# iwbn/flow-supervisor

Measured on AMD Instinct MI355X. Metric: image-pairs/s fwd+bwd, 12 GRU iters, 436x1024, higher is better.
Workload: dtype f32 (bf16x3 products); 1 GPU; RAFT full, 440x1024 (Sintel 436x1024 padded), 12 GRU iters, 4 pairs/GPU, train step = fwd + sequence loss + bwd + RCCL all-reduce + clip + AdamW; global_batch=4, parallelism=dp1, launch=hipGraph replay of the whole step

## Files before the change

### flow_supervisor_amd/_lib.py

```python
import ctypes
import functools
import os
from ctypes import POINTER, Structure, c_double, c_float, c_int, c_int64, c_void_p

import torch

_HERE = os.path.dirname(os.path.abspath(__file__))
LIB_PATH = os.environ.get("FSRAFT_LIB_PATH") or os.path.join(_HERE, "libfsraft.so")
_lib = None

c_float_p = c_void_p


class ConvDesc(Structure):
    _fields_ = [
        ("src", c_void_p * 3), ("srcC", c_int * 3), ("srcld", c_int * 3), ("nsrc", c_int),
        ("wpk", c_void_p), ("bias", c_void_p), ("wpk_split", c_void_p),
        ("B", c_int), ("H", c_int), ("W", c_int), ("KH", c_int), ("KW", c_int), ("N", c_int),
        ("dst", c_void_p * 3), ("dst_bs", c_int64 * 3), ("dst_ps", c_int64 * 3), ("dst_cs", c_int64 * 3),
        ("dst_n0", c_int * 3), ("dst_acc", c_int * 3), ("ndst", c_int),
        ("relu", c_int), ("alpha", c_float),
        ("epi", c_int),
        ("h", c_void_p), ("ldh", c_int), ("z", c_void_p), ("ldz", c_int),
        ("aux1", c_void_p), ("ld1", c_int), ("aux2", c_void_p), ("ld2", c_int), ("hid", c_int),
        ("pre", c_void_p), ("ldpre", c_int),
        ("rmask", c_void_p * 3), ("ldmask", c_int * 3), ("maskc", c_int * 3),
        ("wpk_frag", c_void_p), ("pad_h1", c_int), ("pad_w1", c_int),
        ("ws", c_void_p), ("ws_floats", c_int64),
    ]


class PackJob(Structure):
    _fields_ = [
        ("w", c_void_p * 3), ("rows", c_int * 3), ("npiece", c_int),
        ("wpk", c_void_p),
        ("cin_full", c_int), ("kh", c_int), ("kw", c_int),
        ("srcC", c_int * 3), ("srcOff", c_int * 3), ("nsrc", c_int),
        ("mode", c_int), ("flags", c_int),
        ("scale", c_float), ("accumulate", c_int),
    ]


_PP = POINTER(c_void_p)
_IP = POINTER(c_int)
_S = c_void_p

SIGNATURES = {
    "fsraft_corr_build": [c_void_p, c_void_p, _PP, c_int, c_int, c_int, c_int, c_int, _S],
    "fsraft_corr_unpool_bwd": [_PP, c_int, c_int, c_int, c_int, _S],
    "fsraft_corr_lookup_fwd": [_PP, c_int, c_void_p, c_int64, c_int64, c_int64, c_void_p, c_int, c_int, c_int, c_int, c_int, _S],
    "fsraft_corr_lookup_bwd": [_PP, c_int, c_void_p, c_int64, c_int64, c_int64, c_void_p, c_int, c_int, c_int, c_int, c_int, _S],
    "fsraft_altcorr_fwd": [c_void_p, c_void_p, c_void_p, c_void_p, c_int, c_int, c_int, c_int, c_int, c_int, c_int, c_int, _S],
    "fsraft_altcorr_bwd": [c_void_p, c_void_p, c_void_p, c_void_p, c_void_p, c_void_p, c_int, c_int, c_int, c_int, c_int, c_int, c_int, c_int, _S],
    "fsraft_upsample_fwd": [c_void_p, c_int64, c_int64, c_int64, c_void_p, c_void_p, c_int, c_int, c_int, _S],
    "fsraft_upsample_bwd": [c_void_p, c_int64, c_int64, c_int64, c_void_p, c_void_p, c_void_p, c_void_p, c_void_p, c_int, c_int, c_int, _S],
    "fsraft_upflow8_fwd": [c_void_p, c_void_p, c_int, c_int, c_int, c_int, _S],
    "fsraft_upflow8_bwd": [c_void_p, c_void_p, c_int, c_int, c_int, c_int, _S],
    "fsraft_conv_ktot": [_IP, c_int, c_int, c_int],
    "fsraft_conv_forward": [POINTER(ConvDesc), _S],
    "fsraft_conv_forward_stats": [POINTER(ConvDesc), c_void_p, c_void_p, c_int, POINTER(c_int), _S],
    "fsraft_conv_wgrad": [c_void_p, c_int, c_int, _PP, _IP, _IP, c_int, c_void_p, c_void_p, c_int, c_int, c_int, c_int, c_int, _S],
    "fsraft_conv_wgrad_multi": [_PP, c_int, c_int, c_int, _PP, _IP, _IP, c_int, c_void_p, c_void_p, c_int, c_int, c_int, c_int, c_int, _S],
    "fsraft_conv_small_fwd": [c_void_p, c_int, c_int, c_void_p, c_void_p, c_void_p, c_int64, c_int64, c_int64, c_int, c_int, c_int, c_int, c_int, c_int, _S],
    "fsraft_conv_small_wgrad": [_PP, _PP, c_int, c_int, c_int, c_int, c_void_p, c_void_p, c_int, c_int, c_int, c_int, c_int, c_int, _S],
    "fsraft_conv_small_dgrad": [c_void_p, c_int, c_void_p, c_void_p, c_int, c_void_p, c_int, c_int, c_int, c_int, c_int, c_int, c_int, c_int, _S],
    "fsraft_pack_conv_weights": [POINTER(PackJob), c_int, _S],
    "fsraft_pack_conv_weight": [c_void_p, c_void_p, c_int, c_int, c_int, c_int, _IP, c_int, c_int, c_int, _S],
    "fsraft_set_rec_mfma16": [c_int],
    "fsraft_set_build_kernel": [c_int],
    "fsraft_set_dvol_policy": [c_int],
    "fsraft_set_dvol_box": [c_int],
    "fsraft_set_ktile_exact": [c_int],
    "fsraft_set_lookup_policy": [c_int],
    "fsraft_set_upsample_kernel": [c_int],
    "fsraft_conv_workspace": [c_void_p, c_int64],
    "fsraft_set_arithmetic": [c_int],
    "fsraft_get_arithmetic": [],
    "fsraft_set_tuning": [c_int, c_int],
    "fsraft_adamw_flat": [c_void_p, c_void_p, c_void_p, c_void_p, c_int64, c_void_p, c_void_p, c_float, c_void_p, c_double, c_double, c_float,
                          c_float, c_void_p, c_void_p, _S],
    "fsraft_stream_capture_id": [_S, c_void_p],
    "fsraft_stem_slots": [],
    "fsraft_stem7x7s2_fwd": [c_void_p, c_void_p, c_void_p, c_void_p, c_int, c_int, c_int, c_int, _S],
    "fsraft_stem7x7s2_wgrad": [c_void_p, c_void_p, c_void_p, c_void_p, c_int, c_int, c_int, c_int, _S],
    "fsraft_set_lookup_qb": [c_int],
    "fsraft_set_build_split": [c_int],
    "fsraft_set_gemm_split": [c_int],
    "fsraft_gemm_tn_split": [c_void_p, c_int64, c_int64, c_void_p, c_int64, c_int64, c_void_p, c_int64, c_int64, c_int, c_int, c_int, c_int, c_float, c_int, _S],
    "fsraft_gemm_f32": [c_void_p, c_int64, c_int64, c_void_p, c_int64, c_int64, c_void_p, c_int64, c_int64, c_int, c_int, c_int, c_int, c_int, c_float, c_int, _S],
    "fsraft_nchw_to_nhwc": [c_void_p, c_void_p, c_int, c_int, c_int, c_int, c_int, c_int, _S],
    "fsraft_nhwc_to_nchw": [c_void_p, c_void_p, c_int, c_int, c_int, c_int, c_int, c_int, _S],
    "fsraft_im2col7": [c_void_p, c_int64, c_int64, c_int64, c_void_p, c_int, c_int, c_int, c_int, _S],
    "fsraft_col2im7": [c_void_p, c_int, c_void_p, c_int, c_int, c_int, c_int, _S],
    "fsraft_flow_to_nhwc": [c_void_p, c_int64, c_int64, c_int64, c_void_p, c_int, c_int, c_int, c_int, _S],
    "fsraft_nhwc_to_flow": [c_void_p, c_int, c_int, c_void_p, c_int, c_int, c_int, _S],
    "fsraft_relu_bwd": [c_void_p, c_int, c_void_p, c_int, c_int64, c_int, _S],
    "fsraft_gru_bwd1": [c_void_p, c_void_p, c_void_p, c_void_p, c_void_p, c_void_p, c_int, c_void_p, c_void_p, c_void_p, c_void_p, c_int64, c_int, _S],
    "fsraft_gru_bwd2": [c_void_p, c_void_p, c_void_p, c_void_p, c_int, c_void_p, c_void_p, c_int64, c_int, _S],
    "fsraft_col_sum": [c_void_p, c_int, c_int64, c_int, c_void_p, c_float, _S],
    "fsraft_softmax_rows": [c_void_p, c_int64, c_int, _S],
    "fsraft_softmax_rows_bwd": [c_void_p, c_void_p, c_int64, c_int, _S],
    "fsraft_softmax_rows_rec": [c_void_p, c_int64, c_int, _S],
    "fsraft_softmax_rows_bwd_rec": [c_void_p, c_void_p, c_int64, c_int, _S],
    "fsraft_softmax_rows_pos": [c_void_p, c_void_p, c_int64, c_int64, c_int, c_int, c_int, c_int, c_int, _S],
    "fsraft_softmax_rows_pos_bwd": [c_void_p, c_void_p, c_void_p, c_int64, c_int64, c_int, c_int, c_int, c_int, _S],
    "fsraft_gma_mix_fwd": [c_void_p, c_int, c_void_p, c_int, c_void_p, c_void_p, c_int, c_int64, c_int, _S],
    "fsraft_gma_mix_bwd": [c_void_p, c_int, c_void_p, c_int, c_void_p, c_void_p, c_int, c_void_p, c_int, c_void_p, c_int64, c_int, _S],
    "fsraft_inorm_relu_fwd": [c_void_p, c_void_p, c_void_p, c_int64, c_int, c_float, c_int, _S],
    "fsraft_inorm_relu_bwd": [c_void_p, c_void_p, c_void_p, c_void_p, c_int64, c_int, c_int, _S],
    "fsraft_affine_relu_fwd": [c_void_p, c_void_p, c_void_p, c_void_p, c_int64, c_int, c_int, c_int, _S],
    "fsraft_affine_relu_bwd": [c_void_p, c_void_p, c_void_p, c_void_p, c_void_p, c_void_p, c_void_p, c_int64, c_int, c_int, c_int, _S],
    "fsraft_sequence_loss": [_PP, _PP, POINTER(c_float), c_int, c_int, c_void_p, c_void_p, c_float, c_float, c_int, c_int, c_int, c_void_p, _S],
    "fsraft_corr_pool_pyramid": [_PP, c_int, c_int64, c_int, c_int, _S],
    "fsraft_corr_pool_pyramid_same": [_PP, c_int, c_int64, c_int, c_int, _S],
    "fsraft_corr_lookup_fwd_same": [_PP, c_int, c_void_p, c_int64, c_int64, c_int64, c_void_p, c_int, c_int, c_int, c_int, c_int, _S],
    "fsraft_corr_unpool_same_bwd": [_PP, c_int, c_int64, c_int, c_int, _S],
    "fsraft_corr_lookup_bwd_same": [_PP, c_int, c_void_p, c_int64, c_int64, c_int64, c_void_p, c_int, c_int, c_int, c_int, c_int, _S],
    "fsraft_corr_lookup_dcoords_same": [_PP, c_int, c_void_p, c_int64, c_int64, c_int64, c_void_p, c_int, c_void_p, c_int64, c_int64, c_int64,
                                        c_int, c_int, c_int, c_int, _S],
    "fsraft_set_norm_blocks": [c_int],
    "fsraft_get_tuning": [c_int],
    "fsraft_conv_last_route": [c_int],
    "fsraft_set_wgrad_wide": [c_int],
    "fsraft_conv_wgrad_last_tile": [],
    "fsraft_space_to_depth2": [c_void_p, c_void_p, c_int, c_int, c_int, c_int, c_int, _S],
    "fsraft_forward_interpolate": [c_void_p, c_void_p, c_int, c_int, _S],
    "fsraft_flow_metrics_scratch_bytes": [c_int, c_int, c_int],
    "fsraft_flow_metrics": [c_void_p, c_int64, c_int64, c_int64, c_void_p, c_int64, c_int64, c_int64, c_void_p, c_int64, c_int64,
                            c_int, c_int, c_int, c_void_p, c_void_p, c_void_p, c_int64, _S],
    "fsraft_inorm_relu_cl_fwd": [c_void_p, c_void_p, c_void_p, c_void_p, c_void_p, c_void_p, c_int, c_int, c_int, c_float, c_int, c_int, c_int, _S],
    "fsraft_inorm_relu_cl_bwd": [c_void_p, c_void_p, c_void_p, c_void_p, c_void_p, c_void_p, c_void_p, c_void_p, c_int, c_int, c_int,
                                 c_int, c_int, _S],
    "fsraft_affine_relu_cl_fwd": [c_void_p, c_void_p, c_void_p, c_void_p, c_void_p, c_int64, c_int, c_int, c_int, c_int, _S],
    "fsraft_affine_relu_cl_bwd": [c_void_p, c_void_p, c_void_p, c_void_p, c_void_p, c_void_p, c_void_p, c_void_p, c_void_p, c_int, c_int,
                                  c_int, c_int, c_int, _S],
    "fsraft_axpby": [c_void_p, c_void_p, c_float, c_float, c_int64, _S],
    "fsraft_sum_n": [_PP, c_int, c_void_p, c_int64, c_int, _S],
    "fsraft_bn_fold": [c_void_p, c_void_p, c_void_p, c_void_p, c_void_p, c_float, c_int, c_void_p, c_void_p, c_void_p, c_void_p, _S],
    "fsraft_bn_fold_bwd": [c_void_p, c_int, c_int, c_void_p, c_void_p, c_void_p, c_void_p, c_void_p, c_void_p, _S],
    "fsraft_vol_layout": [c_int, c_int, c_int, _IP],
    "fsraft_corr_build_tiled": [c_void_p, c_void_p, c_void_p, c_int, c_int, c_int, c_int, c_int, _S],
    "fsraft_corr_build_rec": [c_void_p, c_void_p, c_void_p, c_int, c_int, c_int, c_int, c_int, _S],
    "fsraft_corr_lookup_tiled_fwd": [c_void_p, c_int, c_void_p, c_int64, c_int64, c_int64, c_void_p, c_int, c_int, c_int, c_int, c_int, _S],
    "fsraft_corr_lookup_tiled_dcoords": [c_void_p, c_int, c_void_p, c_int64, c_int64, c_int64, c_void_p, c_void_p, c_int64, c_int64, c_int64,
                                         c_int, c_int, c_int, c_int, c_int, _S],
    "fsraft_corr_lookup_dcoords": [_PP, c_int, c_void_p, c_int64, c_int64, c_int64, c_void_p, c_int, c_void_p, c_int64, c_int64, c_int64,
                                   c_int, c_int, c_int, c_int, _S],
    "fsraft_corr_dvol_build": [_PP, _PP, POINTER(c_int64), c_int, c_void_p, c_int, c_int, c_int, c_int, c_int, c_int, c_int, c_int, c_int64,
                               c_int64, c_void_p, c_void_p, _S],
    "fsraft_set_alt_tile": [c_int],
    "fsraft_altcorr_fused_fwd": [c_void_p, _PP, c_int, c_void_p, c_int64, c_int64, c_int64, c_int, c_void_p, c_int, c_int, c_int, c_int, c_int, _S],
    "fsraft_altcorr_fused_dcoords": [c_void_p, _PP, c_int, c_void_p, c_int64, c_int64, c_int64, c_int, c_void_p, c_void_p, c_int64, c_int64,
                                     c_int64, c_int, c_int, c_int, c_int, c_int, _S],
    "fsraft_altcorr_mfma_fwd": [c_void_p, _PP, c_void_p, _PP, c_int, c_void_p, c_int64, c_int64, c_int64, c_int, c_void_p, c_int, c_int, c_int, c_int, c_int, _S],
    "fsraft_corr_f2cat": [c_void_p, c_void_p, c_int, c_int, c_int, c_int, c_int, _S],
    "fsraft_corr_dfmap2": [c_void_p, c_void_p, c_int, c_int, c_int, c_int, c_int, _S],
    "fsraft_corr_f2cat_rec": [c_void_p, c_void_p, c_int, c_int, c_int, c_int, c_int, _S],
    "fsraft_to_records": [c_void_p, c_int64, c_void_p, c_int64, c_int64, c_int, _S],
    "fsraft_gemm_rec_tn": [c_void_p, c_int64, c_int64, c_void_p, c_int64, c_int64, c_void_p, c_int64, c_int64, c_int, c_int, c_int, c_int,
                           c_float, c_int, c_int, _S],
    "fsraft_gemm_rec_nt": [c_void_p, c_int64, c_int64, c_void_p, c_int64, c_int64, c_void_p, c_int64, c_int64, c_int, c_int, c_int, c_int,
                           c_float, c_int, c_int, _S],
    "fsraft_gemm_rec_nt_list": [c_void_p, c_int64, c_int64, c_void_p, c_int64, c_int64, c_void_p, c_int64, c_int64, c_int, c_int, c_int, c_int,
                                c_float, c_int, c_int, c_void_p, c_void_p, c_int, c_int, _S],
    "fsraft_gemm_rec_tn_list": [c_void_p, c_int64, c_int64, c_void_p, c_int64, c_int64, c_void_p, c_int64, c_int64, c_int, c_int, c_int, c_int,
                                c_float, c_int, c_int, c_void_p, c_void_p, c_int, c_int, _S],
    "fsraft_corr_bwd_ktiles": [_PP, POINTER(c_int64), c_int, c_int, c_int, c_int, c_int, c_int, c_int, c_int64, c_int64, c_void_p, c_void_p,
                               c_int, c_void_p, c_void_p, c_void_p, c_int, c_void_p, _S],
}

CONV_ROUTES = {
    1: ("fwd.gemm32", "fp32"), 2: ("fwd.gemm64", "fp32"), 3: ("fwd.gemm64x128", "fp32"), 4: ("fwd.gemm128", "fp32"),
    5: ("fwd.gemm64x64", "fp32"), 6: ("fwd.gemm64x64k16", "fp32"), 7: ("fwd.gemm64x128k16", "fp32"),
    10: ("fwd.patch128x128", "bf16x3"), 11: ("fwd.patch256x128", "bf16x3"), 12: ("fwd.patch128x64", "bf16x3"),
    13: ("fwd.patch256x64", "bf16x3"), 20: ("fwd.halo21", "bf16x3"), 21: ("fwd.halo22", "bf16x3"),
    30: ("fwd.split64x256", "bf16x3"), 31: ("fwd.split256x64", "bf16x3"), 32: ("fwd.split256x128w16", "bf16x3"),
    33: ("fwd.split128x128w8", "bf16x3"), 34: ("fwd.split64x128", "bf16x3"), 35: ("fwd.split128x128", "bf16x3"),
}
CONV_ROUTES.update({c + 100: (n + "+ksplit", a) for c, (n, a) in list(CONV_ROUTES.items()) if c >= 30})
WGRAD_ROUTES = {
    1: ("wgrad.exact32", "fp32"), 2: ("wgrad.exact64x64", "fp32"), 3: ("wgrad.exact128", "fp32"),
    4: ("wgrad.split128", "bf16x3"), 5: ("wgrad.split128S", "bf16x3"), 6: ("wgrad.pack", "bf16x3"),
    7: ("wgrad.patch", "bf16x3"), 8: ("wgrad.multi", "bf16x3"), 9: ("wgrad.multi_w8", "bf16x3"),
}


def load():
    global _lib
    if _lib is not None:
        return _lib
    if not os.path.exists(LIB_PATH):
        raise RuntimeError(
            f"{LIB_PATH} not found: build it with `python -c 'import __graft_entry__ as g; g.build()'` "
            "(or `make -C flow_supervisor_amd/csrc`). There is no CPU/eager fallback for the RAFT hot path.")
    lib = ctypes.CDLL(LIB_PATH)
    for name, argtypes in SIGNATURES.items():
        fn = getattr(lib, name)
        fn.argtypes = argtypes
        fn.restype = c_int
    _lib = lib
    arith = os.environ.get("FSRAFT_ARITHMETIC")
    if arith is not None:
        lib.fsraft_set_arithmetic(int(arith))
    split = os.environ.get("FSRAFT_CONV_SPLIT")
    if split is not None:
        lib.fsraft_set_tuning(3, int(split))
    bsplit = os.environ.get("FSRAFT_BUILD_SPLIT")
    if bsplit is not None:
        lib.fsraft_set_build_split(int(bsplit))
    for kv in filter(None, os.environ.get("FSRAFT_TUNING", "").split(",")):
        key, val = (int(v) for v in kv.split("="))
        if lib.fsraft_set_tuning(key, val) != 0:
            raise RuntimeError(f"FSRAFT_TUNING: key {key} is not a tuning key of this libfsraft (include/fsraft_tuning.h)")
    wsplit = os.environ.get("FSRAFT_WGRAD_SPLIT")
    if wsplit is not None:
        lib.fsraft_set_tuning(4, int(wsplit))
    return lib


def stream():
    return c_void_p(torch.cuda.current_stream().cuda_stream)


def check(rc, what):
    if rc != 0:
        raise RuntimeError(f"libfsraft: {what} failed with status {rc} "
                           f"({'bad argument' if rc == 1 else 'kernel launch error'})")


def ptr(t):
    return c_void_p(t.data_ptr()) if t is not None else c_void_p(0)


def ptr_array(tensors):
    arr = (c_void_p * len(tensors))(*[t.data_ptr() for t in tensors])
    return ctypes.cast(arr, _PP), arr


def int_array(vals):
    return (c_int * len(vals))(*vals)


def require_cuda_f32(*tensors):
    dev = None
    for t in tensors:
        if t is None:
            continue
        if not t.is_cuda:
            raise RuntimeError("fsraft ops need CUDA (ROCm) tensors; the hot path has no CPU implementation")
        if t.dtype != torch.float32:
            raise RuntimeError(f"fsraft ops are fp32-only, got {t.dtype}")
        if dev is None:
            dev = t.device
        elif t.device != dev:
            raise RuntimeError(f"fsraft ops need all tensors on one device, got {dev} and {t.device}")
    if dev is not None and dev.index != torch.cuda.current_device():
        raise RuntimeError(f"fsraft op called with tensors on {dev} while cuda:{torch.cuda.current_device()} is the current device; "
                           f"wrap the call in `with torch.cuda.device({dev.index}):`")


def _first_cuda_device(values):
    for v in values:
        if isinstance(v, torch.Tensor):
            if v.is_cuda:
                return v.device
        elif isinstance(v, (list, tuple)):
            d = _first_cuda_device(v)
            if d is not None:
                return d
    return None


def on_tensor_device(fn):
    @functools.wraps(fn)
    def guarded(*args, **kwargs):
        dev = _first_cuda_device(args)
# ... 8 lines not shown
```

### flow_supervisor_amd/csrc/conv_igemm.hip

```cpp
#include "conv_common.hpp"

namespace {

__device__ __forceinline__ void tile_of_block(int swz, int& bx, int& by) {
  if (!swz) return;
  const int nx = gridDim.x, T = nx * gridDim.y, i = by * nx + bx;
  const int x = i & 7, q = T >> 3, r = T & 7;
  const int t = x * q + (x < r ? x : r) + (i >> 3);
  bx = t % nx; by = t / nx;
}

template <class Cfg>
struct ConvALoader {
  static constexpr int BM = Cfg::BM, BK = Cfg::BK, LD = Cfg::LDA;
  static constexpr int F4 = BK / 4;
  static constexpr int NF4 = BM * F4 / 256;
  static constexpr int NREG = NF4 * 4;
  static constexpr int NCH = NF4;
  const float* p0; const float* p1; const float* p2;
  int C0, C1, C2, ld0, ld1, ld2;
  int cpt0, cpt1, cpt2;
  int taps, KW, PH, PW, H, W;
  int py[NF4], px[NF4];
  int64_t pb[NF4];
// ... 812 lines not shown
      const int mkc = di == 0 ? a.maskc[0] : di == 1 ? a.maskc[1] : a.maskc[2];
      const int64_t b = m / HW, pix = m - b * HW;
      float* o = dp + b * dbs + pix * dps + (int64_t)(n - dn0) * dcs;
      for (int i = 0; i < nv; ++i) {
        float r = v[i] * a.alpha;
        if (a.relu) r = fmaxf(r, 0.f);
        if (dacc) r += o[i * dcs];
        if (mk && n - dn0 + i < mkc && mk[m * ldm + (n - dn0) + i] <= 0.f) r = 0.f;
        o[i * dcs] = r;
      }
    } else if (EPI == EPI_ZR) {
      const bool isz = n < a.hid;
      const int c = isz ? n : n - a.hid;
      if (a.pre) v += gload4(a.pre + m * a.ldpre + n);
#pragma unroll
      for (int i = 0; i < 4; ++i) v[i] = 1.0f / (1.0f + expf(-v[i]));
      if (isz) {
        *reinterpret_cast<f32x4*>(a.dst[0].p + m * a.dst[0].ps + c) = v;
      } else {
        const f32x4 hh = gload4(a.h + m * a.ldh + c);
        *reinterpret_cast<f32x4*>(a.aux2 + m * a.ld2 + c) = v;
        f32x4 rh;
#pragma unroll
        for (int i = 0; i < 4; ++i) rh[i] = v[i] * hh[i];
        *reinterpret_cast<f32x4*>(a.aux1 + m * a.ld1 + c) = rh;
      }
    } else {
      if (a.pre) v += gload4(a.pre + m * a.ldpre + n);
      const f32x4 hh = gload4(a.h + m * a.ldh + n);
      const f32x4 zz = gload4(a.z + m * a.ldz + n);
      f32x4 hn;
#pragma unroll
      for (int i = 0; i < 4; ++i) {
        v[i] = tanhf(v[i]);
        hn[i] = (1.f - zz[i]) * hh[i] + zz[i] * v[i];
      }
      *reinterpret_cast<f32x4*>(a.aux1 + m * a.ld1 + n) = v;
      *reinterpret_cast<f32x4*>(a.dst[0].p + m * a.dst[0].ps + n) = hn;
    }
  }
}

thread_local float* t_reg_ws = nullptr;
thread_local int64_t t_reg_ws_floats = 0;
thread_local float* g_conv_ws = nullptr;
thread_local int64_t g_conv_ws_floats = 0;

int pick_ksplit(int64_t tiles, int KT, int N, int64_t M, int ldw, int bm) {
  int S = 1;
  if (knob.conv_ksplit >= 2) S = knob.conv_ksplit;
  else if (knob.conv_ksplit == -1 && bm == 64 && tiles <= 150 && N <= 256 && KT >= 16) S = (int)((400 + tiles - 1) / tiles);
  else if (knob.conv_ksplit == -1 && bm == 128 && tiles <= 120 && N <= 256 && KT >= (N <= 128 ? 36 : 48)) S = tiles <= 115 ? (int)(230 / tiles) : 2;
  if (S > KT / 6) S = KT / 6;
  if (S > 6) S = 6;
  while (S > 1 && (int64_t)S * M * ldw > g_conv_ws_floats) --S;
  if (S > 1) {
    const int per = (KT + S - 1) / S;
    S = (KT + per - 1) / per;
  }
  return S < 2 ? 1 : S;
}

template <class Cfg>
int launch_conv_split(const ConvArgs& a, int epi, hipStream_t s) {
  const int M = a.B * a.H * a.W;
  dim3 grid(ceil_div(a.N, Cfg::BN), ceil_div(M, Cfg::BM));
  ConvArgsT t;
  const int swz = knob.xcd_swizzle || (grid.x >= 2 && (int64_t)grid.x * grid.y >= 2048);
  const bool buf = knob.conv_buf == 2 || (knob.conv_buf == 1 && Cfg::BM == 64) || Cfg::BN == 256 || Cfg::NT != 256;
  if constexpr (Cfg::LDS_ALLOC >= Cfg::BM * (Cfg::BN + 4) * 4) {
    const int ldw = (a.N + 3) / 4 * 4;
    const bool gru_ok = epi == EPI_PLAIN || (a.N % 4 == 0 && (!a.pre || a.ldpre % 4 == 0));
    const int S = (buf && g_conv_ws && gru_ok && (Cfg::BM == 64 || (Cfg::BM == 128 && Cfg::NT == 512) || knob.conv_ksplit >= 2)) ? pick_ksplit((int64_t)grid.x * grid.y, a.Ktot / 32, a.N, M, ldw, Cfg::BM) : 1;
    if (S > 1) {
      const bool uni_tab = build_ktab_uniform(a, t);
      if (uni_tab || build_ktab(a, t)) {
        ConvArgs& p = t.a;
        p.swz = 0;
        p.ksplit = S;
        p.dst[0] = Dst{g_conv_ws, (int64_t)a.H * a.W * ldw, ldw, 1, 0, 0};
        p.dst[1] = p.dst[2] = p.dst[0];
        p.ndst = 1; p.bias = nullptr; p.relu = 0; p.alpha = 1.0f;
        for (int i = 0; i < 3; ++i) p.rmask[i] = nullptr;
        dim3 g3(grid.x, grid.y, S);
        t_route[0] = route_split<Cfg>() + 100;
        if (uni_tab) hipLaunchKernelGGL((conv_igemm_split_kernel<Cfg, EPI_PLAIN, 2>), g3, dim3(Cfg::NT), 0, s, t);
        else hipLaunchKernelGGL((conv_igemm_split_kernel<Cfg, EPI_PLAIN, 1>), g3, dim3(Cfg::NT), 0, s, t);
        int rc = fs_launch_status();
        if (rc) return rc;
        const int64_t work = (int64_t)M * (ldw / 4);
        const int fb = (int)((work + 255) / 256 < 4096 ? (work + 255) / 256 : 4096);
        with_epi(epi, [&](auto e) { hipLaunchKernelGGL(conv_finish_kernel<decltype(e)::value>, dim3(fb), dim3(256), 0, s, a, g_conv_ws, S, ldw); });
        return fs_launch_status();
      }
    }
  }
  if (buf && build_ktab_uniform(a, t)) {
    t.a.swz = swz;
    t_route[0] = route_split<Cfg>();
    with_epi(epi, [&](auto e) { hipLaunchKernelGGL((conv_igemm_split_kernel<Cfg, decltype(e)::value, 2>), grid, dim3(Cfg::NT), 0, s, t); });
    return fs_launch_status();
  }
  if (buf && build_ktab(a, t)) {
    t.a.swz = swz;
    t_route[0] = route_split<Cfg>();
    with_epi(epi, [&](auto e) { hipLaunchKernelGGL((conv_igemm_split_kernel<Cfg, decltype(e)::value, 1>), grid, dim3(Cfg::NT), 0, s, t); });
    return fs_launch_status();
  }
  if constexpr (Cfg::NT != 256) {
    return -1;
  } else {
  t_route[0] = route_split<Cfg>();
  with_epi(epi, [&](auto e) { hipLaunchKernelGGL((conv_igemm_split_kernel<Cfg, decltype(e)::value>), grid, dim3(256), 0, s, a); });
  return fs_launch_status();
  }
}

template <class Cfg>
int launch_conv_split_plain(const ConvArgs& a, hipStream_t s) {
  const int M = a.B * a.H * a.W;
  dim3 grid(ceil_div(a.N, Cfg::BN), ceil_div(M, Cfg::BM));
  ConvArgsT t;
  if (build_ktab_uniform(a, t)) {
    t_route[0] = route_split<Cfg>();
    hipLaunchKernelGGL((conv_igemm_split_kernel<Cfg, EPI_PLAIN, 2>), grid, dim3(Cfg::NT), 0, s, t);
    return fs_launch_status();
  }
  if (build_ktab(a, t)) {
    t_route[0] = route_split<Cfg>();
    hipLaunchKernelGGL((conv_igemm_split_kernel<Cfg, EPI_PLAIN, 1>), grid, dim3(Cfg::NT), 0, s, t);
    return fs_launch_status();
  }
  return -1;
}

template <class Cfg>
int launch_conv(const ConvArgs& a, int epi, hipStream_t s) {
  const int M = a.B * a.H * a.W;
  dim3 grid(ceil_div(a.N, Cfg::BN), ceil_div(M, Cfg::BM));
  t_route[0] = route_gemm<Cfg>();
  with_epi(epi, [&](auto e) { hipLaunchKernelGGL((conv_igemm_kernel<Cfg, decltype(e)::value>), grid, dim3(256), 0, s, a); });
  return fs_launch_status();
}

#include "conv_patch.inc"

}

extern "C" int fsraft_conv_ktot(const int* srcC, int nsrc, int KH, int KW) {
  if (!srcC || nsrc < 1 || nsrc > 3) return -1;
  return conv_ktot(srcC, nsrc, KH * KW);
}

namespace {
struct StatReq { float* sum; float* sq; int slots; bool done; };
thread_local StatReq t_stat{nullptr, nullptr, 0, false};
template <class Args>
void attach_stats(Args& p, bool want) {
  if (want) { p.st_sum = t_stat.sum; p.st_sq = t_stat.sq; p.st_slots = t_stat.slots; }
}
}

extern "C" int fsraft_conv_forward(const fsraft_conv_desc* d, hipStream_t stream) {
  if (!d || d->nsrc < 1 || d->nsrc > 3 || d->ndst < 1 || d->ndst > 3 || !d->wpk || d->N < 1) return FS_ERR_ARG;
  const bool want_stats = t_stat.sum != nullptr && d->epi == EPI_PLAIN && d->ndst == 1 && !d->relu && d->alpha == 1.0f && !d->dst_acc[0] &&
                          !d->rmask[0] && !d->bias && d->dst_n0[0] == 0 && d->N % 4 == 0;
  if (d->ws && (((uintptr_t)d->ws & 15) || d->ws_floats < 0)) return FS_ERR_ARG;
  t_route[0] = 0;
  g_conv_ws = d->ws ? d->ws : t_reg_ws;
  g_conv_ws_floats = d->ws ? d->ws_floats : t_reg_ws_floats;
  ConvArgs a{};
  if (!fill_srcs(a.src, d->src, d->srcC, d->srcld, d->nsrc)) return FS_ERR_ARG;
  for (int s = 0; s < d->nsrc; ++s) if (d->srcC[s] < 1) return FS_ERR_ARG;
  a.nsrc = d->nsrc;
  a.wpk = d->wpk; a.Ktot = conv_ktot(d->srcC, d->nsrc, d->KH * d->KW); a.bias = d->bias;
  a.B = d->B; a.H = d->H; a.W = d->W; a.KH = d->KH; a.KW = d->KW; a.N = d->N;
  a.PH = d->pad_h1 ? d->pad_h1 - 1 : d->KH / 2; a.PW = d->pad_w1 ? d->pad_w1 - 1 : d->KW / 2;
  if (a.PH < 0 || a.PH >= d->KH || a.PW < 0 || a.PW >= d->KW) return FS_ERR_ARG;
  for (int i = 0; i < 3; ++i) {
    const int j = i < d->ndst ? i : 0;
    a.dst[i] = Dst{d->dst[j], d->dst_bs[j], d->dst_ps[j], d->dst_cs[j], d->dst_n0[j], d->dst_acc[j]};
    if (i < d->ndst && !d->dst[i]) return FS_ERR_ARG;
  }
  a.ndst = d->ndst; a.relu = d->relu; a.alpha = d->alpha;
  a.h = d->h; a.ldh = d->ldh; a.z = d->z; a.ldz = d->ldz; a.aux1 = d->aux1; a.ld1 = d->ld1; a.aux2 = d->aux2; a.ld2 = d->ld2;
  a.hid = d->hid;
  a.pre = d->epi == EPI_PLAIN ? nullptr : d->pre; a.ldpre = d->ldpre;
  if (a.pre && (d->ldpre % 4 != 0 || ((uintptr_t)d->pre & 15))) return FS_ERR_ARG;
  for (int i = 0; i < 3; ++i) {
    const bool on = d->epi == EPI_PLAIN && i < d->ndst && d->rmask[i] != nullptr;
    a.rmask[i] = on ? d->rmask[i] : nullptr; a.ldmask[i] = d->ldmask[i]; a.maskc[i] = d->maskc[i];
    if (on && (d->ldmask[i] % 4 != 0 || ((uintptr_t)d->rmask[i] & 15))) return FS_ERR_ARG;
  }
  a.swz = knob.xcd_swizzle;
  if (d->epi == EPI_ZR && (!d->h || !d->aux1 || !d->aux2 || d->hid * 2 != d->N)) return FS_ERR_ARG;
  if (d->epi == EPI_Q && (!d->h || !d->z || !d->aux1)) return FS_ERR_ARG;
  if (d->epi != EPI_PLAIN && d->epi != EPI_ZR && d->epi != EPI_Q) return FS_ERR_ARG;
  if (knob.conv_patch && knob.conv_patch64 && knob.conv_split == 1 && d->wpk_split && d->epi == EPI_PLAIN && d->KH == 3 && d->KW == 3 &&
      d->N > 32 && d->N <= 64 && (int64_t)d->B * d->H * d->W >= knob.conv_patch_min_m) {
    ConvArgs p = a;
    p.wpk = d->wpk_split;
    attach_stats(p, want_stats);
    const int rc = launch_conv_patch(p, d->epi, stream);
    if (rc >= 0) { t_stat.done = want_stats; return rc; }
  }
  if (knob.conv_halo && knob.conv_split == 1 && d->wpk_frag && d->epi == EPI_PLAIN && d->nsrc == 1 && d->KH == 3 && d->KW == 3 &&
      a.PH == 1 && a.PW == 1 &&
      d->srcC[0] % 4 == 0 && d->srcC[0] > 32 && d->srcC[0] <= 64 && d->N <= 128 && d->N > 32 && d->ndst == 1 &&
      d->dst_cs[0] == 1 && d->dst_n0[0] == 0 && !(d->dst_acc[0] && d->relu) && !a.rmask[0] && d->alpha == 1.0f &&
      (int64_t)d->B * d->H * d->W >= knob.conv_halo_min_m && (int64_t)d->H * d->W * d->srcld[0] * 4 < 0x7fffffff) {
    HaloArgs h{d->src[0], d->srcld[0], d->srcC[0], reinterpret_cast<const char*>(d->wpk_frag), d->bias,
               d->dst[0], d->dst_bs[0], d->dst_ps[0], d->N, d->B, d->H, d->W, d->relu, d->dst_acc[0], nullptr, nullptr, 0};
    attach_stats(h, want_stats);
    t_stat.done = want_stats;
    t_route[0] = d->N > 64 ? 21 : 20;
    return d->N > 64 ? launch_halo<2, 2>(h, stream) : launch_halo<2, 1>(h, stream);
  }
  if (d->N <= 32 && d->epi == EPI_PLAIN) return launch_conv<Cfg32>(a, d->epi, stream);
  if (d->N <= 64 && d->epi == EPI_PLAIN && !(knob.conv_split && d->wpk_split && knob.conv_buf)) return launch_conv<Cfg64>(a, d->epi, stream);
  const int M = d->B * d->H * d->W;
  if (knob.conv_split && d->wpk_split && d->N > 32) {
    a.wpk = d->wpk_split;
    const bool narrow = knob.conv_buf != 0 || (int64_t)ceil_div(d->N, 128) * ceil_div(M, 128) < 400;
    if (knob.conv_patch && knob.conv_split == 1 && d->KH * d->KW > 1 && d->N > 64 && M >= knob.conv_patch_min_m) {
      ConvArgs p = a;
      attach_stats(p, want_stats);
      const int rc = launch_conv_patch(p, d->epi, stream);
      if (rc >= 0) { t_stat.done = want_stats; return rc; }
    }
    if (knob.conv_split == 5 || (knob.conv_split == 1 && knob.conv_n256 && d->N >= 256 &&
                              ceil_div(d->N, 256) * 256 <= ceil_div(d->N, 128) * 128))
      return launch_conv_split<SCfgN256>(a, d->epi, stream);
    if (knob.conv_split == 1 && knob.conv_n64 && d->N <= 64 && d->epi == EPI_PLAIN && M >= knob.conv_n64_min_m) {
      const int rc = launch_conv_split_plain<SCfg256N64>(a, stream);
      if (rc >= 0) return rc;
    }
    if (knob.conv_split == 1 && ((knob.conv_w8 == 1 && d->N >= 192 && d->N <= 512 && M >= 16384) || knob.conv_w8 == 2) && d->N >= 192) {
      const int rc = launch_conv_split<SCfg256W16>(a, d->epi, stream);
      if (rc >= 0) return rc;
    }
    if (knob.conv_w8 && knob.conv_split == 1 && (int64_t)ceil_div(d->N, 128) * ceil_div(M, 128) >= knob.conv_w8_min) {
      const int rc = launch_conv_split<SCfg128W8>(a, d->epi, stream);
      if (rc >= 0) return rc;
    }
    if (knob.conv_split == 3) return launch_conv_split<SCfgM64>(a, d->epi, stream);
    if (knob.conv_split == 4) return launch_conv_split<SCfg128>(a, d->epi, stream);
    return narrow ? launch_conv_split<SCfgM64>(a, d->epi, stream) : launch_conv_split<SCfg128>(a, d->epi, stream);
  }
  if (knob.conv_tile == 3) return launch_conv<Cfg6464>(a, d->epi, stream);
  if (knob.conv_tile == 4) return launch_conv<Cfg6464K16>(a, d->epi, stream);
  if (knob.conv_tile == 5) return launch_conv<CfgM64K16>(a, d->epi, stream);
  if (knob.conv_tile == 2) return launch_conv<CfgM64>(a, d->epi, stream);
  if (knob.conv_tile == 1) return launch_conv<Cfg128>(a, d->epi, stream);
  if ((int64_t)ceil_div(d->N, 128) * ceil_div(M, 128) < 512) return launch_conv<CfgM64>(a, d->epi, stream);
  return launch_conv<Cfg128>(a, d->epi, stream);
}

extern "C" int fsraft_conv_forward_stats(const fsraft_conv_desc* d, float* sum, float* sq, int slots, int* done, hipStream_t stream) {
  if (!sum || !sq || slots < 1 || !done) return FS_ERR_ARG;
  t_stat = StatReq{sum, sq, slots, false};
  const int rc = fsraft_conv_forward(d, stream);
  *done = (rc == FS_OK && t_stat.done) ? 1 : 0;
  t_stat = StatReq{nullptr, nullptr, 0, false};
  return rc;
}


extern "C" int fsraft_conv_workspace(float* ws, int64_t floats) {
  if (ws && (((uintptr_t)ws & 15) || floats < 0)) return FS_ERR_ARG;
  t_reg_ws = ws;
  t_reg_ws_floats = ws ? floats : 0;
  return FS_OK;
}
```

### flow_supervisor_amd/csrc/conv_patch.inc

```
constexpr int PT_TW = 32, PT_BN = 128;
constexpr int PT_GMAX = 32;

struct PatchArgs {
  ConvArgs a;
  int ngroups;
  int tx;
  unsigned gtab[PT_GMAX];
  int cpt[3];
};

template <int EPI, int KH, int KW, int PT_TH, int BN = PT_BN>
__global__ __launch_bounds__(PT_TH * 64) void conv_patch_kernel(const PatchArgs args) {
  constexpr int PT_NT = PT_TH * 64, TN = BN / 64;
  using PCfg = SplitCfg<PT_TH * 32, BN, PT_TH / 2, 2, 2, true, PT_NT>;
  constexpr int TAPS = KH * KW, PHh = KH / 2, PWh = KW / 2;
  constexpr int PH = PT_TH + KH - 1, PW = PT_TW + KW - 1, ROWS = PH * PW;
  constexpr int PPITCH = 144;
  constexpr int PT_PLANE = ROWS * PPITCH;
  constexpr int PT_NCHP = (ROWS * 8 + PT_NT - 1) / PT_NT;
  constexpr int EPI_BYTES = PT_TH * 32 * (BN + 4) * 4, RING = 2 * PT_PLANE + 2 * BN * 128;
  __shared__ __attribute__((aligned(16))) char lds[RING > EPI_BYTES ? RING : EPI_BYTES];
  const ConvArgs& a = args.a;
  const int lane = threadIdx.x & 63, wave = __builtin_amdgcn_readfirstlane((int)(threadIdx.x >> 6));
  const int wm = wave >> 1, wn = wave & 1, l31 = lane & 31, lh = lane >> 5;
  const int n0 = blockIdx.x * BN;
  const int tile = blockIdx.y, tpi = args.tx * ((a.H + PT_TH - 1) / PT_TH);
  const int b = tile / tpi, trem = tile % tpi;
  const int y0 = (trem / args.tx) * PT_TH, x0 = (trem % args.tx) * PT_TW;
  const auto* gtab = (const unsigned __attribute__((address_space(4)))*)(
      (const char __attribute__((address_space(4)))*)__builtin_amdgcn_kernarg_segment_ptr() + offsetof(PatchArgs, gtab));
  const int NG = args.ngroups;

  unsigned ppix[PT_NCHP];
  const unsigned part16 = (threadIdx.x & 7) * 16;
#pragma unroll
  for (int j = 0; j < PT_NCHP; ++j) {
    const int row = (threadIdx.x + PT_NT * j) >> 3;
    const int y = y0 - PHh + row / PW, x = x0 - PWh + row % PW;
    const bool ok = row < ROWS && (unsigned)y < (unsigned)a.H && (unsigned)x < (unsigned)a.W;
    ppix[j] = ok ? (unsigned)((b * a.H + y) * a.W + x) : 0x7fffffffu;
  }
  constexpr int NCHW = BN * 8 / PT_NT;
  unsigned vbw[NCHW];
#pragma unroll
  for (int j = 0; j < NCHW; ++j) {
    const int e = threadIdx.x + PT_NT * j;
    vbw[j] = (e >> 3) < a.N - n0 ? (unsigned)((e >> 3) * a.Ktot * 4 + (e & 7) * 16) : FS_OOB;
  }
  const char* wbase = uni_ptr(reinterpret_cast<const char*>(a.wpk) + (int64_t)n0 * a.Ktot * 4);

  struct Group { const float* base; unsigned ld4, soff, crem4; int kt0, step; };
  auto group = [&](int g) {
    const unsigned e = gtab[__builtin_amdgcn_readfirstlane(g < NG ? g : NG - 1)];
    const unsigned src = e & 3u, c = (e >> 2) & 255u, crem = (e >> 10) & 63u;
    const bool s1 = src >= 1, s2 = src >= 2;
    Group r;
    r.base = uni_ptr(a.src[0].p + (s1 ? a.src[1].p - a.src[0].p : 0) + (s2 ? a.src[2].p - a.src[1].p : 0));
    r.ld4 = uni((unsigned)(a.src[0].ld + (s1 ? a.src[1].ld - a.src[0].ld : 0) + (s2 ? a.src[2].ld - a.src[1].ld : 0)) * 4u);
    r.soff = c * 128u; r.crem4 = crem * 4u;
    r.kt0 = (int)(e >> 16);
    r.step = args.cpt[0] + (s1 ? args.cpt[1] - args.cpt[0] : 0) + (s2 ? args.cpt[2] - args.cpt[1] : 0);
    return r;
  };
  float rp[PT_NCHP * 4];
  auto fetch_patch = [&](const Group& gr) {
    const __amdgpu_buffer_rsrc_t rs = make_rsrc(gr.base, 0x7fffffffu);
    const unsigned cok = part16 < gr.crem4 ? 0u : 0x80000000u;
#pragma unroll
    for (int j = 0; j < PT_NCHP; ++j) {
      const unsigned voff = ppix[j] == 0x7fffffffu ? FS_OOB : ((ppix[j] * gr.ld4 + part16) | cok);
      const f32x4 f = __builtin_bit_cast(f32x4, __builtin_amdgcn_raw_buffer_load_b128(rs, voff, gr.soff, 0));
      rp[4 * j] = f[0]; rp[4 * j + 1] = f[1]; rp[4 * j + 2] = f[2]; rp[4 * j + 3] = f[3];
    }
  };
  auto stage_patch = [&](char* plane) {
#pragma unroll
    for (int j = 0; j < PT_NCHP; ++j) {
      const int e = threadIdx.x + PT_NT * j;
      if ((e >> 3) < ROWS) stage_convert<PPITCH>(plane, e, rp + 4 * j);
    }
  };
  const __amdgpu_buffer_rsrc_t rsW = make_rsrc(wbase, 0x7fffffffu);
  float rw[NCHW * 4];
  auto fetch_w = [&](int kt) {
    const int ku = __builtin_amdgcn_readfirstlane(kt);
#pragma unroll
    for (int j = 0; j < NCHW; ++j) {
      const f32x4 f = __builtin_bit_cast(f32x4, __builtin_amdgcn_raw_buffer_load_b128(rsW, ku < 0 ? FS_OOB : vbw[j], ku < 0 ? 0u : (unsigned)ku * 128u, 0));
      rw[4 * j] = f[0]; rw[4 * j + 1] = f[1]; rw[4 * j + 2] = f[2]; rw[4 * j + 3] = f[3];
    }
  };
  auto stage_w = [&](char* bt) {
#pragma unroll
    for (int j = 0; j < NCHW; ++j) stage_copy<128>(bt, threadIdx.x + PT_NT * j, rw + 4 * j);
  };

  f32x16 acc[2][TN];
#pragma unroll
  for (int i = 0; i < 2; ++i)
#pragma unroll
    for (int j = 0; j < TN; ++j)
#pragma unroll
      for (int r = 0; r < 16; ++r) acc[i][j][r] = 0.f;
  char* plane0 = lds;
  char* plane1 = lds + PT_PLANE;
  char* bt0 = lds + 2 * PT_PLANE;
  char* bt1 = bt0 + BN * 128;

  const int rb = wn * (BN / 2) + l31;
  const int la_off = (2 * wm * PW + l31) * PPITCH + lh * 16;
  auto compute = [&](const char* plane, const char* bt, int dy, int dx) {
    const char* Bs = bt + rb * 128;
#pragma unroll
    for (int s = 0; s < 2; ++s) {
      bf16x8 ah[2], al[2], bh[TN], bl[TN];
#pragma unroll
      for (int mt = 0; mt < 2; ++mt) {
        ah[mt] = *reinterpret_cast<const bf16x8*>(plane + la_off + ((dy + mt) * PW + dx) * PPITCH + (2 * s) * 16);
        al[mt] = *reinterpret_cast<const bf16x8*>(plane + la_off + ((dy + mt) * PW + dx) * PPITCH + (4 + 2 * s) * 16);
      }
      const int obh = slot_offset<128>(rb, 2 * s + lh) - rb * 128, obl = slot_offset<128>(rb, 4 + 2 * s + lh) - rb * 128;
#pragma unroll
      for (int nt = 0; nt < TN; ++nt) {
        bh[nt] = *reinterpret_cast<const bf16x8*>(Bs + nt * 32 * 128 + obh);
        bl[nt] = *reinterpret_cast<const bf16x8*>(Bs + nt * 32 * 128 + obl);
      }
#pragma unroll
      for (int mt = 0; mt < 2; ++mt)
#pragma unroll
        for (int nt = 0; nt < TN; ++nt) acc[mt][nt] = __builtin_amdgcn_mfma_f32_32x32x16_bf16(al[mt], bh[nt], acc[mt][nt], 0, 0, 0);
#pragma unroll
      for (int mt = 0; mt < 2; ++mt)
#pragma unroll
        for (int nt = 0; nt < TN; ++nt) acc[mt][nt] = __builtin_amdgcn_mfma_f32_32x32x16_bf16(ah[mt], bl[nt], acc[mt][nt], 0, 0, 0);
#pragma unroll
      for (int mt = 0; mt < 2; ++mt)
#pragma unroll
        for (int nt = 0; nt < TN; ++nt) acc[mt][nt] = __builtin_amdgcn_mfma_f32_32x32x16_bf16(ah[mt], bh[nt], acc[mt][nt], 0, 0, 0);
    }
  };

  Group gc = group(0);
  fetch_patch(gc);
  fetch_w(gc.kt0);
  stage_patch(plane0);
  stage_w(bt0);
  Group gn = group(1);
  if (NG > 1) fetch_patch(gn);
  fetch_w(TAPS > 1 ? gc.kt0 + gc.step : (NG > 1 ? gn.kt0 : -1));
  __syncthreads();
  for (int g = 0; g < NG; ++g) {
#pragma unroll
    for (int t = 0; t < TAPS; ++t) {
      const int i = g * TAPS + t;
      char* btc = (i & 1) ? bt1 : bt0;
      char* btn = (i & 1) ? bt0 : bt1;
      compute((g & 1) ? plane1 : plane0, btc, t / KW, t % KW);
      stage_w(btn);
      {
        const int t2 = t + 2;
        int kt;
        if (t2 < TAPS) kt = gc.kt0 + t2 * gc.step;
        else kt = g + 1 < NG ? gn.kt0 + (t2 - TAPS) * gn.step : -1;
        if (TAPS == 1) {
          const Group g2 = group(g + 2);
          kt = g + 2 < NG ? g2.kt0 : -1;
        }
        fetch_w(kt);
      }
      if (t == TAPS - 1 && g + 1 < NG) {
        stage_patch((g & 1) ? plane0 : plane1);
        gc = gn;
        gn = group(g + 2);
        if (g + 2 < NG) fetch_patch(gn);
      }
      __syncthreads();
    }
  }
  conv_epilogue_lds<PCfg, EPI, PT_NT, true>(a, acc, 0, n0, reinterpret_cast<float*>(lds), true, b, y0, x0);
}

template <int KH, int KW, int TH>
int launch_conv_patch_t(const PatchArgs& p, int epi, dim3 grid, hipStream_t s) {
  t_route[0] = (TH == 8 ? 11 : 10) + (KH == 3 && KW == 3 && p.a.N <= 64 ? 2 : 0);
  if constexpr (KH == 3 && KW == 3) {
    if (p.a.N <= 64) {
      hipLaunchKernelGGL((conv_patch_kernel<EPI_PLAIN, 3, 3, TH, 64>), grid, dim3(TH * 64), 0, s, p);
      return fs_launch_status();
    }
  }
  with_epi(epi, [&](auto e) { hipLaunchKernelGGL((conv_patch_kernel<decltype(e)::value, KH, KW, TH>), grid, dim3(TH * 64), 0, s, p); });
  return fs_launch_status();
}

int launch_conv_patch(const ConvArgs& a, int epi, hipStream_t s) {
  const bool k33 = a.KH == 3 && a.KW == 3, k15 = a.KH == 1 && a.KW == 5, k51 = a.KH == 5 && a.KW == 1;
  if (!(k33 || k15 || k51) || a.PH != a.KH / 2 || a.PW != a.KW / 2 || !epilogue_rows_ok_host(a)) return -1;
  PatchArgs p;
  p.a = a; p.a.swz = 0;
  int ng = 0, kt = 0;
  const int taps = a.KH * a.KW;
  for (int sidx = 0; sidx < 3; ++sidx) p.cpt[sidx] = 1;
  for (int sidx = 0; sidx < a.nsrc; ++sidx) {
    const int C = a.src[sidx].C, cpt = (C + 31) / 32;
    p.cpt[sidx] = cpt;
    if ((int64_t)a.B * a.H * a.W * a.src[sidx].ld * 4 >= (int64_t)0x7fffffff) return -1;
    for (int c = 0; c < cpt; ++c) {
      if (ng >= PT_GMAX || kt + c >= (1 << 16)) return -1;
      const int crem = C - c * 32 < 32 ? C - c * 32 : 32;
      p.gtab[ng++] = (unsigned)sidx | (unsigned)c << 2 | (unsigned)crem << 10 | (unsigned)(kt + c) << 16;
    }
    kt += taps * cpt;
  }
  if (kt * 32 != a.Ktot || ng < 1) return -1;
  for (int g = ng; g < PT_GMAX; ++g) p.gtab[g] = p.gtab[ng - 1];
  p.ngroups = ng;
  p.tx = ceil_div(a.W, PT_TW);
  const int bn = a.N <= 64 ? 64 : PT_BN;
  if (bn == 64 && !(k33 && epi == EPI_PLAIN)) return -1;
  const int64_t wg8 = (int64_t)ceil_div(a.N, bn) * p.tx * ceil_div(a.H, 8) * a.B;
  if (bn == 64 && wg8 >= 200 && knob.conv_patch64 == 1) return -1;
  if (wg8 >= 200 && !(bn == 64 && knob.conv_patch64 == 2)) {
    dim3 grid(ceil_div(a.N, bn), p.tx * ceil_div(a.H, 8) * a.B);
    if (k33) return launch_conv_patch_t<3, 3, 8>(p, epi, grid, s);
    if (k15) return launch_conv_patch_t<1, 5, 8>(p, epi, grid, s);
    return launch_conv_patch_t<5, 1, 8>(p, epi, grid, s);
  }
  const bool small_grid_33 = k33 && a.N > 128 && (int64_t)ceil_div(a.N, 128) * ceil_div(a.B * a.H * a.W, 128) > 120;
  if (knob.conv_patch != 2 && bn != 64 && !small_grid_33) return -1;
  dim3 grid(ceil_div(a.N, bn), p.tx * ceil_div(a.H, 4) * a.B);
  if (k33) return launch_conv_patch_t<3, 3, 4>(p, epi, grid, s);
  if (k15) return launch_conv_patch_t<1, 5, 4>(p, epi, grid, s);
  return launch_conv_patch_t<5, 1, 4>(p, epi, grid, s);
}
```

### include/fsraft_tuning.h

```cpp
#ifndef FSRAFT_TUNING_H
#define FSRAFT_TUNING_H

#ifdef __cplusplus
extern "C" {
#endif

enum fsraft_tuning_key {
  FSRAFT_KEY_CONV_TILE = 0,
  FSRAFT_KEY_WGRAD_TILE = 1,
  FSRAFT_KEY_WGRAD_BLOCKS = 2,
  FSRAFT_KEY_CONV_ARITH = 3,
  FSRAFT_KEY_WGRAD_ARITH = 4,
  FSRAFT_KEY_CONV_BUF = 5,
  FSRAFT_KEY_XCD_SWIZZLE = 7,
  FSRAFT_KEY_WGRAD_BUF = 8,
  FSRAFT_KEY_CONV_N256 = 9,
  FSRAFT_KEY_WGRAD_MULTI = 10,
  FSRAFT_KEY_WGRAD_BLOCKS_MULTI = 11,
  FSRAFT_KEY_CONV_UNIFORM = 12,
  FSRAFT_KEY_CONV_W8 = 13,
  FSRAFT_KEY_CONV_W8_MIN = 14,
  FSRAFT_KEY_WGRAD_W8 = 15,
  FSRAFT_KEY_WGRAD_PACK = 16,
  FSRAFT_KEY_WGRAD_BLOCKS_PACK = 17,
  FSRAFT_KEY_CONV_N64 = 18,
  FSRAFT_KEY_CONV_N64_MIN_M = 19,
  FSRAFT_KEY_CONV_HALO = 20,
  FSRAFT_KEY_CONV_HALO_MIN_M = 21,
  FSRAFT_KEY_WGRAD_XCD = 22,
  FSRAFT_KEY_CONV_PATCH = 26,
  FSRAFT_KEY_WGRAD_PATCH = 27,
  FSRAFT_KEY_CONV_PATCH64 = 28,
  FSRAFT_KEY_WGRAD_PATCH1 = 29,
  FSRAFT_KEY_CONV_PATCH_MIN_M = 31,
  FSRAFT_KEY_CONV_KSPLIT = 32
};
int fsraft_set_tuning(int key, int value);
int fsraft_get_tuning(int key);
int fsraft_conv_last_route(int which);
int fsraft_set_wgrad_wide(int mode);
int fsraft_conv_wgrad_last_tile(void);
int fsraft_set_build_split(int on);
int fsraft_set_build_kernel(int which);
int fsraft_set_lookup_policy(int aux);
int fsraft_set_ktile_exact(int levels);
int fsraft_set_upsample_kernel(int v4);
int fsraft_set_dvol_box(int on);
int fsraft_set_dvol_policy(int policy);
int fsraft_set_gemm_split(int on);
int fsraft_set_lookup_qb(int qb);
int fsraft_set_norm_blocks(int target_workgroups);
int fsraft_set_rec_mfma16(int on);
int fsraft_set_alt_tile(int on);

#ifdef __cplusplus
}
#endif
#endif
```

Measured before the change: 111.9 image-pairs/s.

## Deepen weight prefetch and interleave patch loads across taps in patch conv

Adds a look-ahead variant of the patch convolution kernel. It keeps several register sets of weight tiles in flight (two by default, for the 8-row, 128-wide tile) instead of one. The next channel-group's patch fetch and LDS staging are split into per-tap pieces spread over the tap loop, rather than done in one burst at the end of a group. The aim is to hide global-load latency and smooth the memory traffic per barrier step. The cost is more registers per thread, which can lower occupancy, plus extra template instantiations. A runtime setter and a tuning mode that forces the 8-row tile are also added.

```diff
diff --git a/flow_supervisor_amd/_lib.py b/flow_supervisor_amd/_lib.py
--- a/flow_supervisor_amd/_lib.py
+++ b/flow_supervisor_amd/_lib.py
@@ -122,6 +122,7 @@
     "fsraft_get_tuning": [c_int],
     "fsraft_conv_last_route": [c_int],
     "fsraft_set_wgrad_wide": [c_int],
+    "fsraft_set_patch_ahead": [c_int],
     "fsraft_conv_wgrad_last_tile": [],
     "fsraft_space_to_depth2": [c_void_p, c_void_p, c_int, c_int, c_int, c_int, c_int, _S],
     "fsraft_forward_interpolate": [c_void_p, c_void_p, c_int, c_int, _S],
diff --git a/flow_supervisor_amd/csrc/conv_igemm.hip b/flow_supervisor_amd/csrc/conv_igemm.hip
--- a/flow_supervisor_amd/csrc/conv_igemm.hip
+++ b/flow_supervisor_amd/csrc/conv_igemm.hip
@@ -988,6 +988,12 @@
   return conv_ktot(srcC, nsrc, KH * KW);
 }
 
+extern "C" int fsraft_set_patch_ahead(int mode) {
+  if (mode < 0 || mode > 3) return FS_ERR_ARG;
+  g_patch_ahead = mode;
+  return FS_OK;
+}
+
 namespace {
 struct StatReq { float* sum; float* sq; int slots; bool done; };
 thread_local StatReq t_stat{nullptr, nullptr, 0, false};
diff --git a/flow_supervisor_amd/csrc/conv_patch.inc b/flow_supervisor_amd/csrc/conv_patch.inc
--- a/flow_supervisor_amd/csrc/conv_patch.inc
+++ b/flow_supervisor_amd/csrc/conv_patch.inc
@@ -9,7 +9,7 @@
   int cpt[3];
 };
 
-template <int EPI, int KH, int KW, int PT_TH, int BN = PT_BN>
+template <int EPI, int KH, int KW, int PT_TH, int BN = PT_BN, int AH = 0>
 __global__ __launch_bounds__(PT_TH * 64) void conv_patch_kernel(const PatchArgs args) {
   constexpr int PT_NT = PT_TH * 64, TN = BN / 64;
   using PCfg = SplitCfg<PT_TH * 32, BN, PT_TH / 2, 2, 2, true, PT_NT>;
@@ -63,9 +63,9 @@
     return r;
   };
   float rp[PT_NCHP * 4];
-  auto fetch_patch = [&](const Group& gr) {
+  auto fetch_patch = [&](const Group& gr, bool valid) {
     const __amdgpu_buffer_rsrc_t rs = make_rsrc(gr.base, 0x7fffffffu);
-    const unsigned cok = part16 < gr.crem4 ? 0u : 0x80000000u;
+    const unsigned cok = valid && part16 < gr.crem4 ? 0u : 0x80000000u;
 #pragma unroll
     for (int j = 0; j < PT_NCHP; ++j) {
       const unsigned voff = ppix[j] == 0x7fffffffu ? FS_OOB : ((ppix[j] * gr.ld4 + part16) | cok);
@@ -73,26 +73,35 @@
       rp[4 * j] = f[0]; rp[4 * j + 1] = f[1]; rp[4 * j + 2] = f[2]; rp[4 * j + 3] = f[3];
     }
   };
+  auto fetch_patch_part = [&](const Group& gr, bool valid, int j) {
+    const __amdgpu_buffer_rsrc_t rs = make_rsrc(gr.base, 0x7fffffffu);
+    const unsigned cok = valid && part16 < gr.crem4 ? 0u : 0x80000000u;
+    const unsigned voff = ppix[j] == 0x7fffffffu ? FS_OOB : ((ppix[j] * gr.ld4 + part16) | cok);
+    const f32x4 f = __builtin_bit_cast(f32x4, __builtin_amdgcn_raw_buffer_load_b128(rs, voff, gr.soff, 0));
+    rp[4 * j] = f[0]; rp[4 * j + 1] = f[1]; rp[4 * j + 2] = f[2]; rp[4 * j + 3] = f[3];
+  };
+  auto stage_patch_part = [&](char* plane, int j) {
+    const int e = threadIdx.x + PT_NT * j;
+    if ((e >> 3) < ROWS) stage_convert<PPITCH>(plane, e, rp + 4 * j);
+  };
   auto stage_patch = [&](char* plane) {
 #pragma unroll
-    for (int j = 0; j < PT_NCHP; ++j) {
-      const int e = threadIdx.x + PT_NT * j;
-      if ((e >> 3) < ROWS) stage_convert<PPITCH>(plane, e, rp + 4 * j);
-    }
+    for (int j = 0; j < PT_NCHP; ++j) stage_patch_part(plane, j);
   };
   const __amdgpu_buffer_rsrc_t rsW = make_rsrc(wbase, 0x7fffffffu);
-  float rw[NCHW * 4];
-  auto fetch_w = [&](int kt) {
+  constexpr int NSET = AH > 0 ? AH : 1;
+  float rw[NSET][NCHW * 4];
+  auto fetch_w = [&](int kt, int set) {
     const int ku = __builtin_amdgcn_readfirstlane(kt);
 #pragma unroll
     for (int j = 0; j < NCHW; ++j) {
       const f32x4 f = __builtin_bit_cast(f32x4, __builtin_amdgcn_raw_buffer_load_b128(rsW, ku < 0 ? FS_OOB : vbw[j], ku < 0 ? 0u : (unsigned)ku * 128u, 0));
-      rw[4 * j] = f[0]; rw[4 * j + 1] = f[1]; rw[4 * j + 2] = f[2]; rw[4 * j + 3] = f[3];
-    }
-  };
-  auto stage_w = [&](char* bt) {
-#pragma unroll
-    for (int j = 0; j < NCHW; ++j) stage_copy<128>(bt, threadIdx.x + PT_NT * j, rw + 4 * j);
+      rw[set][4 * j] = f[0]; rw[set][4 * j + 1] = f[1]; rw[set][4 * j + 2] = f[2]; rw[set][4 * j + 3] = f[3];
+    }
+  };
+  auto stage_w = [&](char* bt, int set) {
+#pragma unroll
+    for (int j = 0; j < NCHW; ++j) stage_copy<128>(bt, threadIdx.x + PT_NT * j, rw[set] + 4 * j);
   };
 
   f32x16 acc[2][TN];
@@ -140,57 +149,111 @@
     }
   };
 
-  Group gc = group(0);
-  fetch_patch(gc);
-  fetch_w(gc.kt0);
-  stage_patch(plane0);
-  stage_w(bt0);
-  Group gn = group(1);
-  if (NG > 1) fetch_patch(gn);
-  fetch_w(TAPS > 1 ? gc.kt0 + gc.step : (NG > 1 ? gn.kt0 : -1));
-  __syncthreads();
-  for (int g = 0; g < NG; ++g) {
-#pragma unroll
-    for (int t = 0; t < TAPS; ++t) {
-      const int i = g * TAPS + t;
-      char* btc = (i & 1) ? bt1 : bt0;
-      char* btn = (i & 1) ? bt0 : bt1;
-      compute((g & 1) ? plane1 : plane0, btc, t / KW, t % KW);
-      stage_w(btn);
-      {
-        const int t2 = t + 2;
-        int kt;
-        if (t2 < TAPS) kt = gc.kt0 + t2 * gc.step;
-        else kt = g + 1 < NG ? gn.kt0 + (t2 - TAPS) * gn.step : -1;
-        if (TAPS == 1) {
-          const Group g2 = group(g + 2);
-          kt = g + 2 < NG ? g2.kt0 : -1;
+  if constexpr (AH == 0) {
+    Group gc = group(0);
+    fetch_patch(gc, true);
+    fetch_w(gc.kt0, 0);
+    stage_patch(plane0);
+    stage_w(bt0, 0);
+    Group gn = group(1);
+    if (NG > 1) fetch_patch(gn, true);
+    fetch_w(TAPS > 1 ? gc.kt0 + gc.step : (NG > 1 ? gn.kt0 : -1), 0);
+    __syncthreads();
+    for (int g = 0; g < NG; ++g) {
+#pragma unroll
+      for (int t = 0; t < TAPS; ++t) {
+        const int i = g * TAPS + t;
+        char* btc = (i & 1) ? bt1 : bt0;
+        char* btn = (i & 1) ? bt0 : bt1;
+        compute((g & 1) ? plane1 : plane0, btc, t / KW, t % KW);
+        stage_w(btn, 0);
+        {
+          const int t2 = t + 2;
+          int kt;
+          if (t2 < TAPS) kt = gc.kt0 + t2 * gc.step;
+          else kt = g + 1 < NG ? gn.kt0 + (t2 - TAPS) * gn.step : -1;
+          if (TAPS == 1) {
+            const Group g2 = group(g + 2);
+            kt = g + 2 < NG ? g2.kt0 : -1;
+          }
+          fetch_w(kt, 0);
         }
-        fetch_w(kt);
-      }
-      if (t == TAPS - 1 && g + 1 < NG) {
-        stage_patch((g & 1) ? plane0 : plane1);
-        gc = gn;
-        gn = group(g + 2);
-        if (g + 2 < NG) fetch_patch(gn);
-      }
-      __syncthreads();
+        if (t == TAPS - 1 && g + 1 < NG) {
+          stage_patch((g & 1) ? plane0 : plane1);
+          gc = gn;
+          gn = group(g + 2);
+          if (g + 2 < NG) fetch_patch(gn, true);
+        }
+        __syncthreads();
+      }
+    }
+  } else {
+    static_assert(TAPS > AH + 1, "a weight tile's look-ahead must not reach beyond the next chunk");
+    constexpr int UN = AH / (TAPS % AH == 0 ? AH : (AH % (TAPS % AH) == 0 ? TAPS % AH : 1));
+    static_assert((UN * TAPS) % AH == 0, "register sets must line up across trips");
+    Group gc = group(0);
+    fetch_patch(gc, true);
+#pragma unroll
+    for (int j = 0; j < AH; ++j) fetch_w(gc.kt0 + j * gc.step, j);
+    stage_patch(plane0);
+    stage_w(bt0, 0);
+    Group gn = group(1);
+    fetch_w(gc.kt0 + AH * gc.step, 0);
+    fetch_patch(gn, NG > 1);
+    Group gf = gn;
+    __syncthreads();
+    for (int g0 = 0; g0 < NG; g0 += UN) {
+#pragma unroll
+      for (int u = 0; u < UN; ++u) {
+        const int g = g0 + u;
+        if (u > 0 && g >= NG) break;
+#pragma unroll
+        for (int t = 0; t < TAPS; ++t) {
+          const int i = g * TAPS + t;
+          const int set = (u * TAPS + t + 1) % AH;
+          char* btc = (i & 1) ? bt1 : bt0;
+          char* btn = (i & 1) ? bt0 : bt1;
+          compute((g & 1) ? plane1 : plane0, btc, t / KW, t % KW);
+          stage_w(btn, set);
+          const int t2 = t + AH + 1;
+          fetch_w(t2 < TAPS ? gc.kt0 + t2 * gc.step : (g + 1 < NG ? gn.kt0 + (t2 - TAPS) * gn.step : -1), set);
+          if (t == 0) gf = group(g + 2);
+#pragma unroll
+          for (int j = t; j < PT_NCHP; j += TAPS) {
+            stage_patch_part((g & 1) ? plane0 : plane1, j);
+            fetch_patch_part(gf, g + 2 < NG, j);
+          }
+          if (t == TAPS - 1) { gc = gn; gn = gf; }
+          __syncthreads();
+        }
+      }
     }
   }
   conv_epilogue_lds<PCfg, EPI, PT_NT, true>(a, acc, 0, n0, reinterpret_cast<float*>(lds), true, b, y0, x0);
+}
+
+int g_patch_ahead = 1;
+int patch_ahead_default(int TH, int bn) { return TH == 8 && bn == PT_BN ? 2 : 0; }
+
+template <int KH, int KW, int TH, int AH>
+int launch_conv_patch_a(const PatchArgs& p, int epi, dim3 grid, hipStream_t s) {
+  if constexpr (KH == 3 && KW == 3) {
+    if (p.a.N <= 64) {
+      hipLaunchKernelGGL((conv_patch_kernel<EPI_PLAIN, 3, 3, TH, 64, AH>), grid, dim3(TH * 64), 0, s, p);
+      return fs_launch_status();
+    }
+  }
+  with_epi(epi, [&](auto e) { hipLaunchKernelGGL((conv_patch_kernel<decltype(e)::value, KH, KW, TH, PT_BN, AH>), grid, dim3(TH * 64), 0, s, p); });
+  return fs_launch_status();
 }
 
 template <int KH, int KW, int TH>
 int launch_conv_patch_t(const PatchArgs& p, int epi, dim3 grid, hipStream_t s) {
   t_route[0] = (TH == 8 ? 11 : 10) + (KH == 3 && KW == 3 && p.a.N <= 64 ? 2 : 0);
-  if constexpr (KH == 3 && KW == 3) {
-    if (p.a.N <= 64) {
-      hipLaunchKernelGGL((conv_patch_kernel<EPI_PLAIN, 3, 3, TH, 64>), grid, dim3(TH * 64), 0, s, p);
-      return fs_launch_status();
-    }
-  }
-  with_epi(epi, [&](auto e) { hipLaunchKernelGGL((conv_patch_kernel<decltype(e)::value, KH, KW, TH>), grid, dim3(TH * 64), 0, s, p); });
-  return fs_launch_status();
+  const int ah = g_patch_ahead == 1 ? patch_ahead_default(TH, p.a.N <= 64 ? 64 : PT_BN) : g_patch_ahead;
+  if (ah == 2) return launch_conv_patch_a<KH, KW, TH, 2>(p, epi, grid, s);
+  if (ah == 3) return launch_conv_patch_a<KH, KW, TH, 3>(p, epi, grid, s);
+  return launch_conv_patch_a<KH, KW, TH, 0>(p, epi, grid, s);
 }
 
 int launch_conv_patch(const ConvArgs& a, int epi, hipStream_t s) {
@@ -220,7 +283,7 @@
   if (bn == 64 && !(k33 && epi == EPI_PLAIN)) return -1;
   const int64_t wg8 = (int64_t)ceil_div(a.N, bn) * p.tx * ceil_div(a.H, 8) * a.B;
   if (bn == 64 && wg8 >= 200 && knob.conv_patch64 == 1) return -1;
-  if (wg8 >= 200 && !(bn == 64 && knob.conv_patch64 == 2)) {
+  if ((wg8 >= 200 && !(bn == 64 && knob.conv_patch64 == 2)) || knob.conv_patch == 3) {
     dim3 grid(ceil_div(a.N, bn), p.tx * ceil_div(a.H, 8) * a.B);
     if (k33) return launch_conv_patch_t<3, 3, 8>(p, epi, grid, s);
     if (k15) return launch_conv_patch_t<1, 5, 8>(p, epi, grid, s);
diff --git a/include/fsraft_tuning.h b/include/fsraft_tuning.h
--- a/include/fsraft_tuning.h
+++ b/include/fsraft_tuning.h
@@ -40,6 +40,7 @@
 int fsraft_conv_last_route(int which);
 int fsraft_set_wgrad_wide(int mode);
 int fsraft_conv_wgrad_last_tile(void);
+int fsraft_set_patch_ahead(int mode);
 int fsraft_set_build_split(int on);
 int fsraft_set_build_kernel(int which);
 int fsraft_set_lookup_policy(int aux);
```

Measured after the change: 112.4 image-pairs/s, median of 6. Within noise of the previous version (+0.4%).
